# Guivernoir/ICS-WT-PhysicsEngine

Hardware: AMD Instinct MI355X
Metric: reactor-zone-steps/sec (higher is better)
Workload: dtype f64

## Files before the change

### ics-wt-physicsengine_amd/csrc/wt_device.hpp

```cpp
#pragma once
#include <hip/hip_runtime.h>
#include <stdint.h>
#include <type_traits>
#include "wt_sensors.hpp"
#include "wt_ctl.hpp"
#include "wt_inj.hpp"
#include "wt_alm.hpp"
#include "wt_det.hpp"
#include "wt_act.hpp"
#include "wt_dst.hpp"
#include "wt_scr.hpp"

namespace wt {

#ifdef WT_STAMPS
constexpr int WT_DIAG_SLOTS = 16;
#else
constexpr int WT_DIAG_SLOTS = 8;
#endif

constexpr int SPH = 0, SCL = 1, STT = 2;
#define WT_RARE(x) __builtin_expect(!!(x), 0)
#define WT_USUAL(x) __builtin_expect(!!(x), 1)
constexpr double RTOL = 1e-6, ATOL = 1e-8;
// ... 1220 lines not shown
            const double kd = k_diag(k, n.k_lo, khi_up);
            put(SPH, 2, row_pH(k, mix3(n.k_lo, khi_up, kd, n.H_lo, n.H_hi, b.H), b.H, b.iw));
            put(SCL, 2, row_Cl(k, mix3(n.k_lo, khi_up, kd, n.C_lo, n.C_hi, y[SCL]), y[SCL], kphi));
            put(STT, 2, row_T(k, mix3(n.k_lo, khi_up, kd, n.T_lo, Tx_hi, y[STT]), y[STT]));
        }
    }
}

template <bool ROW, int SP>
__device__ __forceinline__ void fd_col_reduce(const Lane &L, const FdCols &c, double &maxd, double &scale)
{
    maxd = -1.0; scale = 0.0;
#pragma unroll
    for (int q = 0; q < 3; ++q) {
        const bool dep_nb = (q == SP) || (SP == STT);
        const bool dep_own = dep_nb || (q == SCL && SP == SPH);
        if (!dep_own) continue;
        double d_lo = 0, s_lo = 0, d_hi = 0, s_hi = 0;
        if (dep_nb) {
            d_lo = from_lo<ROW, 1>(L, c.D[q][2]); s_lo = from_lo<ROW, 1>(L, c.S[q][2]);
            d_hi = from_hi<ROW, 1>(L, c.D[q][0]); s_hi = from_hi<ROW, 1>(L, c.S[q][0]);
        }
        if (dep_nb && L.has_lo && fabs(d_lo) > maxd) { maxd = fabs(d_lo); scale = s_lo; }
        if (fabs(c.D[q][1]) > maxd) { maxd = fabs(c.D[q][1]); scale = c.S[q][1]; }
        if (dep_nb && L.has_hi && fabs(d_hi) > maxd) { maxd = fabs(d_hi); scale = s_hi; }
    }
}

__device__ __forceinline__ double fd_step(double y, double fac, double ysc)
{
    return __dadd_rn(__dadd_rn(y, __dmul_rn(fac, ysc)), -y);
}

template <bool ROW, int SP, class KC>
__device__ __forceinline__ void num_jac_species(const Lane &L, const KC &kc, const RK &k, const double y[3], const double f[3],
                                                const ZoneProps &b, const FdBase &nb, double &fac, FdCols &cols, bool &bad, double &badval)
{
    const double fs = (f[SP] >= 0) ? 1.0 : -1.0;
    const double ysc = fs * fmax(ATOL, fabs(y[SP]));
    double h = fd_step(y[SP], fac, ysc);
    while (WT_RARE(h == 0)) { fac *= 10; h = fd_step(y[SP], fac, ysc); }
    fd_species_pass<ROW, SP>(L, kc, k, y, f, b, nb, h, true, true, cols, bad, badval);
    double maxd, scl;
    fd_col_reduce<ROW, SP>(L, cols, maxd, scl);
    const bool small = maxd < rc::NJ_REJECT * scl;
    if (WT_RARE(__ballot(small) != 0ull)) {
        const double nf = 10 * fac;
        const double hn = fd_step(y[SP], nf, ysc);
        FdCols c2;
        fd_species_pass<ROW, SP>(L, kc, k, y, f, b, nb, hn, small, false, c2, bad, badval);
        double md2, sc2;
        fd_col_reduce<ROW, SP>(L, c2, md2, sc2);
        const bool upd = small && (maxd * sc2 < md2 * scl);
        if (upd) { fac = nf; h = hn; maxd = md2; scl = sc2; }
        const int iu = upd ? 1 : 0;
        const int iu_lo = __shfl_up(iu, 1, 64), iu_hi = __shfl_down(iu, 1, 64);
        const bool upd_lo = L.has_lo && (iu_lo != 0), upd_hi = L.has_hi && (iu_hi != 0);
#pragma unroll
        for (int q = 0; q < 3; ++q) {
            if (upd_lo) cols.D[q][0] = c2.D[q][0];
            if (upd) cols.D[q][1] = c2.D[q][1];
            if (upd_hi) cols.D[q][2] = c2.D[q][2];
        }
    }
    const double h_lo = from_lo<ROW, 1>(L, h), h_hi = from_hi<ROW, 1>(L, h);
    const double ih0 = L.has_lo ? rcp(h_lo) : 0.0, ih1 = rcp(h), ih2 = L.has_hi ? rcp(h_hi) : 0.0;
#pragma unroll
    for (int q = 0; q < 3; ++q) { cols.D[q][0] *= ih0; cols.D[q][1] *= ih1; cols.D[q][2] *= ih2; }
    const bool sm = maxd < rc::NJ_SMALL * scl, bg = maxd > rc::NJ_BIG * scl;
    if (sm) fac *= 10;
    if (bg) fac *= 0.1;
    fac = fmax(fac, rc::NJ_MINF);
}

template <bool ROW, class KTP>
__device__ __forceinline__ void num_jac(const Lane &L, const RKStore &ks, KTP ktab, const double y[3], const double f[3],
                                        double fac[3], bool &have_fac, Jac &J, bool &bad, double &badval, bool &t_dense)
{
    if (!have_fac) { fac[0] = fac[1] = fac[2] = rc::NJ_F0; have_fac = true; }
    FdCols cols;
    ZoneProps b;
    FdBase nb;
    {
        const KT ct = load_kt(ktab());
        const PropT bpt = prop_T(ct, y[STT]);
        b.kT = bpt.kT; b.rho = bpt.rho;
    }
    {
        const KP cp = load_kp(ktab());
        const RK k = fetch_reactor(ks);
        const PropPH bpp = prop_pH(cp, k, y[SPH]);
        b.H = bpp.H; b.iw = bpp.iw; b.phi = bpp.phi; b.bpos = bpp.bpos;
        nb = fd_base<ROW>(L, k, y, b);
        num_jac_species<ROW, SPH>(L, cp, k, y, f, b, nb, fac[SPH], cols, bad, badval);
#pragma unroll
        for (int r = 0; r < 3; ++r) J.pp[r] = cols.D[SPH][r];
        J.cp = cols.D[SCL][1];
    }
    {
        const RK k = fetch_reactor(ks);
        num_jac_species<ROW, SCL>(L, 0, k, y, f, b, nb, fac[SCL], cols, bad, badval);
#pragma unroll
        for (int r = 0; r < 3; ++r) J.cc[r] = cols.D[SCL][r];
    }
    {
        const KT ct = load_kt(ktab());
        const RK k = fetch_reactor(ks);
        num_jac_species<ROW, STT>(L, ct, k, y, f, b, nb, fac[STT], cols, bad, badval);
#pragma unroll
        for (int r = 0; r < 3; ++r) { J.tt[r] = cols.D[STT][r]; J.pt[r] = cols.D[SPH][r]; J.ct[r] = cols.D[SCL][r]; }
        t_dense = jac_t_dense(J) || (ct.dense_bias != 0.0);
    }
}

template <bool ROW, int LV = 6>
__device__ __forceinline__ double rms3(const Lane &L, const double x[3], const double sc[3])
{
    double s = 0.0;
#pragma unroll
    for (int q = 0; q < 3; ++q) { const double v = x[q] * rcp(sc[q]); s += v * v; }
    return sqrt_k(div_by(seg_sum<ROW, LV>(L, s), L.d3n));
}

__device__ __forceinline__ double ulp_above(double t)
{
    return __longlong_as_double(__double_as_longlong(t) + 1) - t;
}

__device__ __forceinline__ double predict_factor(double h_abs, bool have_old, double h_abs_old,
                                                 double error_norm, double error_norm_old)
{
    double mult = 1.0;
    const double ie = rcp(error_norm);
    if (have_old && error_norm != 0) mult = h_abs * rcp(h_abs_old) * root4(error_norm_old * ie);
    return fmin(1.0, mult) * root4(ie);
}

struct Flag {
    uint32_t &w; const uint32_t m;
    __device__ __forceinline__ operator bool() const { return (w & m) != 0u; }
    __device__ __forceinline__ Flag &operator=(bool v) { w = v ? (w | m) : (w & ~m); return *this; }
    __device__ __forceinline__ Flag &operator=(const Flag &o) { return *this = (bool)o; }
    __device__ __forceinline__ Flag &operator|=(bool v) { w = v ? (w | m) : w; return *this; }
};

enum Phase : int {
    PH_OUTER_BEGIN = 0,
    PH_INIT_STEP,
    PH_F1,
    PH_STEP_BEGIN,
    PH_ATTEMPT,
    PH_NEWTON,
    PH_ERR_REFINE,
    PH_FNEW,
    PH_DONE
};

struct SolverCounters { int nfev, njev, nlu, nsteps, nrej; };

__device__ __forceinline__ void lane_geometry(int n, Lane &L)
{
    const int lane = threadIdx.x & 63;
    const int seg = lane / n;
    L.n = n; L.z = lane - seg * n;
    L.base = seg * n;
    L.a_me = lane << 3; L.xrow = nullptr;
    L.has_lo = L.z > 0; L.has_hi = L.z < n - 1;
#pragma unroll
    for (int l = 0; l < 7; ++l) {
        L.m_lo[l] = (L.z - (1 << l) >= 0) ? ~0u : 0u;
        L.m_hi[l] = (L.z + (1 << l) < n) ? ~0u : 0u;
        asm("" : "+v"(L.m_lo[l]));
        asm("" : "+v"(L.m_hi[l]));
    }
    L.segmask = ((n >= 64) ? ~0ull : ((1ull << n) - 1ull)) << L.base;
    {
        int top = 1;
        while (2 * top < n) top *= 2;
        const bool up = L.z >= top, has = up || (L.z + top < n);
        L.m_pt = has ? ~0u : 0u;
        asm("" : "+v"(L.m_pt));
    }
    L.d3n = {(double)(3 * n), 1.0 / (double)(3 * n)};
    L.d9n = {(double)(9 * n), 1.0 / (double)(9 * n)};
}

__device__ __forceinline__ bool lane_setup(int64_t r0, int64_t r1, int n, int R, Lane &L, int64_t &r)
{
    lane_geometry(n, L);
    const int seg = (threadIdx.x & 63) / n;
    r = r0 + (int64_t)blockIdx.x * R + seg;
    return (seg < R) && (r < r1);
}

template <int LV> struct LdsMap {
    static constexpr int RK_DOUBLES = RK_UNI * rk_maxr(LV) + rk_lane_doubles(LV);
    static constexpr int HIST_DOUBLES = rk_maxr(LV);
    static constexpr int F_DOUBLES = FSlots<LV>::LDS_SLOTS * 64;
    static constexpr int IO_DOUBLES = (int)((sizeof(wts::StepIO) + 7) / 8);
    static constexpr int TAIL_DOUBLES = F_DOUBLES > IO_DOUBLES ? F_DOUBLES : IO_DOUBLES;
    static constexpr int X_OFF = RK_DOUBLES + HIST_DOUBLES, X_DOUBLES = 64;
    static constexpr int F_OFF = (X_OFF + X_DOUBLES + 1) & ~1;
    static constexpr int TOTAL = F_OFF + TAIL_DOUBLES;
    static_assert(X_OFF >= (LV >= 2 ? (1 << (LV - 2)) : 0), "reads below the exchange row must stay inside the allocation");
};

typedef const __attribute__((address_space(4))) StepArgs *ArgPtr;
__device__ __forceinline__ ArgPtr fresh(ArgPtr p)
{
    asm volatile("" : "+s"(p));
    return p;
}

__device__ __forceinline__ int queue_resolve(ArgPtr a, int ticket)
{
    const int n_groups = a->n_groups;
    if (ticket < n_groups) return n_groups - 1 - ticket;
    const unsigned long long want = (unsigned long long)(unsigned)(ticket + 1);
    unsigned long long *slot = a->q_slots + (ticket - n_groups) % a->q_cap;
    for (int spin = 0; spin < (1 << 22); ++spin) {
        const unsigned long long w = __hip_atomic_load(slot, __ATOMIC_RELAXED, __HIP_MEMORY_SCOPE_AGENT);
        if ((w >> 32) == want) return (int)(w & 0xffffffffull);
        __builtin_amdgcn_s_sleep(2);
    }
    __hip_atomic_store(a->q_ctrl + Q_ERROR, 1, __ATOMIC_RELAXED, __HIP_MEMORY_SCOPE_AGENT);
    return -1;
}

__device__ __forceinline__ void queue_push(ArgPtr a, int group)
{
    int32_t *ctrl = a->q_ctrl;
    const int p = __hip_atomic_fetch_add(ctrl + Q_TAIL, 1, __ATOMIC_RELAXED, __HIP_MEMORY_SCOPE_AGENT);
    const unsigned long long w = ((unsigned long long)(unsigned)(a->n_groups + p + 1) << 32) | (unsigned)group;
    __hip_atomic_store(a->q_slots + p % a->q_cap, w, __ATOMIC_RELAXED, __HIP_MEMORY_SCOPE_AGENT);
    __hip_atomic_fetch_add(ctrl + Q_AVAIL, 1, __ATOMIC_RELEASE, __HIP_MEMORY_SCOPE_AGENT);
}

__device__ __forceinline__ int queue_next(ArgPtr pa, int own, bool hold, bool &exchanged)
{
    ArgPtr a = fresh(pa);
    const bool lane0 = (threadIdx.x & 63) == 0;
    int ticket = -1;
    if (lane0 && !(own >= 0 && hold)) {
        int32_t *avail = a->q_ctrl + Q_AVAIL;
        do {
            const int old = __hip_atomic_fetch_add(avail, -1, __ATOMIC_RELAXED, __HIP_MEMORY_SCOPE_AGENT);
            if (old > 0) { ticket = __hip_atomic_fetch_add(a->q_ctrl + Q_HEAD, 1, __ATOMIC_RELAXED, __HIP_MEMORY_SCOPE_AGENT); break; }
            __hip_atomic_fetch_add(avail, 1, __ATOMIC_RELAXED, __HIP_MEMORY_SCOPE_AGENT);
        } while (__hip_atomic_load(avail, __ATOMIC_RELAXED, __HIP_MEMORY_SCOPE_AGENT) > 0);
    }
    ticket = __builtin_amdgcn_readfirstlane(ticket);
    exchanged = ticket >= 0;
    if (ticket < 0) return own;
    if (own >= 0) {
        asm volatile("s_waitcnt vmcnt(0)" ::: "memory");
        __builtin_amdgcn_fence(__ATOMIC_RELEASE, "agent");
        asm volatile("s_waitcnt vmcnt(0)" ::: "memory");
    }
    int next = -1;
    if (lane0) {
        if (own >= 0) queue_push(a, own);
        next = queue_resolve(a, ticket);
    }
    return __builtin_amdgcn_readfirstlane(next);
}

template <bool ROW, int NS>
__device__ __forceinline__ void rhs_points(const Lane &L, const RKStore &ks, ArgPtr pa, const double (*y)[3], double (*F)[3], bool *bad)
{
    PropPH pp[NS]; PropT pt[NS];
    {
        ArgPtr a = fresh(pa);
        const KP c = load_kp(&a->kt);
        const RK k = fetch_reactor(ks);
        double x[NS];
#pragma unroll
        for (int s = 0; s < NS; ++s) x[s] = y[s][SPH];
        prop_pH_n<NS>(c, k, x, pp);
    }
    __builtin_amdgcn_sched_barrier(0);
    {
        ArgPtr a = fresh(pa);
        const KT c = load_kt(&a->kt);
        double x[NS];
#pragma unroll
        for (int s = 0; s < NS; ++s) x[s] = y[s][STT];
        prop_T_n<NS>(c, x, pt);
#pragma unroll
        for (int s = 0; s < NS; ++s) bad[s] = pt[s].bad;
    }
    {
        const RK k = fetch_reactor(ks);
#pragma unroll
        for (int s = 0; s < NS; ++s)
            rhs_rows<ROW>(L, k, pp[s].H, pp[s].iw, pp[s].bpos, pt[s].kT * pp[s].phi, pt[s].rho, y[s][SCL], y[s][STT], F[s]);
    }
}

template <int LV, bool ROW>
__device__ __forceinline__ void run_item(ArgPtr pa, const Lane &L, double *lds, int group, int step0, int cnt)
{
    using M = LdsMap<LV>;
    ArgPtr a = fresh(pa);
    const int n_zones = L.n, R = a->R;
    const int lane = threadIdx.x & 63, seg = lane / n_zones;
    const int64_t q_first = (int64_t)group * R;
    const int64_t q_end = a->q_ctrl ? a->N : a->r1;
    const bool present = (seg < R) && (q_first + seg < q_end);
    const int64_t r = present ? (int64_t)a->perm[q_first + seg] : 0;
    const int64_t idx = r * n_zones + L.z;
    const double dt = a->dt;
    const int step_limit = a->step_limit, sens_on = a->sens.on, plc_on = a->sens.plc_on;
    const bool want_diag = a->wave_diag != nullptr;
    const RKStore ks = {lds + seg, lds + RK_UNI * rk_maxr(LV) + lane, rk_maxr(LV), L.m_lo[0], L.m_hi[0], rk_lane_in_lds(LV)};
    int *hist0 = reinterpret_cast<int *>(lds + M::RK_DOUBLES);
    int *rix = hist0 + rk_maxr(LV);
    double *lds_factors = lds + M::F_OFF;
    wts::StepIO &io = *reinterpret_cast<wts::StepIO *>(lds_factors);

    double y0[3] = {7.0, 1.0, 20.0};
    double f[3] = {0, 0, 0};
    double t_out = 0;
    double dH = 0, dR = 0, dK = 0, badval = 0;
    double flow_used = 0;
    uint32_t st = 0;
    bool frozen = !present, f_valid = false, wrote_k = false, raised = false;
    int steps_done = 0, reads_done = 0, cost_acc = 0;
    SolverCounters last_cnt = {0, 0, 0, 0, 0};
    int diag_trips = 0, diag_newton = 0;
#ifdef WT_STAMPS
    int diag_fact = 0, diag_jac = 0, diag_f3 = 0;
#define WT_COUNT(c) ++(c)
#else
    constexpr int diag_fact = 0, diag_jac = 0, diag_f3 = 0;
#define WT_COUNT(c) do { } while (0)
#endif
#ifdef WT_STAMPS
    long long sec[8] = {0, 0, 0, 0, 0, 0, 0, 0}; long long tprev = __builtin_amdgcn_s_memtime();
#define WT_STAMP(i) do { const long long tn_ = __builtin_amdgcn_s_memtime(); sec[i] += tn_ - tprev; tprev = tn_; } while (0)
#else
#define WT_STAMP(i) do { } while (0)
#endif
    const long long clk0 = want_diag ? __builtin_amdgcn_s_memtime() : 0, wall0 = want_diag ? __builtin_amdgcn_s_memrealtime() : 0;
    if (present) {
        st = a->status[r];
        if (st & (ST_T_RANGE | ST_T_RANGE_POST)) frozen = true;
        y0[SPH] = a->pH[idx]; y0[SCL] = a->Cl[idx]; y0[STT] = a->T[idx];
        t_out = a->time[r];
        const double *bc = a->sched ? a->sched + (int64_t)(a->first_step + step0) * NB * a->N : a->bc;
        RK k0; load_reactor(a->par, bc, a->N, r, n_zones, k0); mask_reactor_for_lane(L, k0);
        park_reactor(ks, k0);
        if (sens_on && L.z == 0) hist0[seg] = a->sens.hist_value ? a->sens.hist_pos[r] : 0;
        if (L.z == 0) rix[seg] = (int)r;
    }

    for (int k = 0; k < cnt; ++k) {
        bool stepped = false;
        if (!frozen) {
          if (WT_RARE(seg_any(L, !(isfinite(y0[0]) && isfinite(y0[1]) && isfinite(y0[2]))))) { st |= ST_NONFINITE; frozen = true; }
          else {
            double yc[3], W[3][3];
            double aux[3] = {0, 0, 0};
            constexpr bool HELD = LV <= 5;
            typedef Held<HELD> AReg64;
            AReg64 Qa[3][3], y_old_a[3], sol_t_old_a, sol_h_a;
#pragma unroll
            for (int q = 0; q < 3; ++q) { y_old_a[q].init(); Qa[q][0].init(); Qa[q][1].init(); Qa[q][2].init(); }
            sol_t_old_a.init(); sol_h_a.init();
            Jac J;
            JacA<(LV <= 4)> ja; ja.init();
            FStore<LV> F;
            F.cell = (LdsDouble2 *)lds_factors + lane;
            uint32_t fl = 1u << 4;
            Flag have_fac{fl, 1u << 0}, have_old{fl, 1u << 1}, have_old_l{fl, 1u << 2}, have_sol{fl, 1u << 3}, current_jac{fl, 1u << 4},
                 have_lu{fl, 1u << 5}, rejected{fl, 1u << 6}, keep_h{fl, 1u << 7}, have_norm_old{fl, 1u << 8}, have_rate{fl, 1u << 9},
                 bad{fl, 1u << 10}, failed{fl, 1u << 11}, fv{fl, 1u << 12}, need_jac{fl, 1u << 13},
                 limit_hit{fl, 1u << 16}, pend_f{fl, 1u << 17}, jac_after_fnew{fl, 1u << 18},
                 j_dense{fl, 1u << 19};
            fv = f_valid;
            AReg64 fac_a[3]; fac_a[0].init(); fac_a[1].init(); fac_a[2].init();
            double t = t_out, t_bound = t_out + dt, max_step = fmin(dt, 10.0);
            double h = 0, t_new = 0, h_abs = 0, h_abs_l = 0, min_step = 0;
            AReg64 h_abs_old_a, err_old_a, h_abs_old_l_a, err_old_l_a;
            h_abs_old_a.init(); err_old_a.init(); h_abs_old_l_a.init(); err_old_l_a.init();
            int kk = 0, n_iter = 0; double dW_norm_old = 0, rate = 0;
            double error_norm = 0, safety = 0;
            double d0 = 0, d1 = 0, h0 = 0;
            SolverCounters cnt_s = {0, 0, 0, 0, 0};
            int attempts = 0;
            int badstage = 0;
            int phase = PH_OUTER_BEGIN;
#pragma unroll
            for (int q = 0; q < 3; ++q) { yc[q] = y0[q]; W[0][q] = W[1][q] = W[2][q] = 0.0; }

            auto initial_step_first_half = [&]() {
                double sc[3];
#pragma unroll
                for (int q = 0; q < 3; ++q) sc[q] = ATOL + fabs(yc[q]) * RTOL;
                d0 = rms3<ROW, LV>(L, yc, sc); d1 = rms3<ROW, LV>(L, f, sc);
                h0 = (d0 < 1e-5 || d1 < 1e-5) ? 1e-6 : 0.01 * d0 * rcp(d1);
                h0 = fmin(h0, fabs(t_bound - t));
#pragma unroll
                for (int q = 0; q < 3; ++q) aux[q] = yc[q] + h0 * f[q];
            };
            auto reject_step = [&]() {
                const double fct = predict_factor(h_abs_l, have_old_l, h_abs_old_l_a.get(), error_norm, err_old_l_a.get());
                h_abs_l *= fmax(MIN_FACTOR, safety * fct);
                have_lu = false; rejected = true; cnt_s.nrej++;
                phase = PH_ATTEMPT;
            };
            auto accept_step = [&]() {
                const bool recompute_jac = (n_iter > 2) && have_rate && (rate > 1e-3);
                double fct = predict_factor(h_abs_l, have_old_l, h_abs_old_l_a.get(), error_norm, err_old_l_a.get());
                fct = fmin(MAX_FACTOR, safety * fct);
                if (!recompute_jac && fct < 1.2) fct = 1.0; else have_lu = false;
                h_abs_old_a.set(h_abs);
                err_old_a.set(error_norm);
                have_old = true;
                h_abs = h_abs_l * fct;
                const KZ kz = lit_kz(); const KA ka = lit_ka();
#pragma unroll
                for (int q = 0; q < 3; ++q) {
                    const double z0 = kz.T00 * W[0][q] + kz.T01 * W[1][q] + kz.T02 * W[2][q];
                    const double z1 = kz.T10 * W[0][q] + kz.T11 * W[1][q] + kz.T12 * W[2][q];
                    const double z2 = W[0][q] + W[1][q];
                    y_old_a[q].set(yc[q]);
                    Qa[q][0].set(z0 * ka.P[0] + z1 * ka.P[3] + z2 * ka.P[6]);
                    Qa[q][1].set(z0 * ka.P[1] + z1 * ka.P[4] + z2 * ka.P[7]);
                    Qa[q][2].set(z0 * ka.P[2] + z1 * ka.P[5] + z2 * ka.P[8]);
                    yc[q] = yc[q] + z2;
                }
                sol_t_old_a.set(t); sol_h_a.set(t_new - t); have_sol = true;
                t = t_new;
                cnt_s.nsteps++; cnt_s.nfev++;
                pend_f = true; fv = false;
                current_jac = recompute_jac;
                const bool more = (t - t_bound) < 0;
                if (recompute_jac || !more) { jac_after_fnew = recompute_jac; phase = PH_FNEW; }
                else phase = PH_STEP_BEGIN;
            };

            if (fv) {
                cnt_s.nfev++;
                phase = PH_INIT_STEP;
            }

            WT_STAMP(0);
            while (true) {
                if (__ballot(phase != PH_DONE) == 0ull) break;
                if (phase == PH_INIT_STEP) {
                    initial_step_first_half();
                    phase = PH_F1;
                }
                if (phase == PH_STEP_BEGIN) {
                    min_step = 10 * fabs(ulp_above(t));
                    if (h_abs > max_step) { h_abs_l = max_step; have_old_l = false; }
                    else if (h_abs < min_step) { h_abs_l = min_step; have_old_l = false; }
                    else { h_abs_l = h_abs; have_old_l = have_old; h_abs_old_l_a.set(h_abs_old_a.get()); err_old_l_a.set(err_old_a.get()); }
                    rejected = false; keep_h = false;
                    phase = PH_ATTEMPT;
                }
                if (phase == PH_ATTEMPT) {
                    if (!keep_h) {
                        if (WT_RARE(step_limit > 0 && attempts >= step_limit)) { failed = true; limit_hit = true; phase = PH_DONE; }
                        else if (WT_RARE(h_abs_l < min_step)) { failed = true; phase = PH_DONE; }
                        else {
                            attempts++;
                            h = h_abs_l;
                            t_new = t + h;
                            if (t_new - t_bound > 0) t_new = t_bound;
                            h = t_new - t;
                            h_abs_l = fabs(h);
                        }
                    }
                    if (phase == PH_ATTEMPT) {
                        keep_h = false;
                        double Z0[3][3];
                        if (!have_sol) {
#pragma unroll
                            for (int s = 0; s < 3; ++s)
#pragma unroll
                                for (int q = 0; q < 3; ++q) Z0[s][q] = 0.0;
                        } else {
                            const double sol_t_old = sol_t_old_a.get(), isol = rcp(sol_h_a.get());
                            double Q[3][3], y_old[3];
#pragma unroll
                            for (int q = 0; q < 3; ++q) { y_old[q] = y_old_a[q].get(); Q[q][0] = Qa[q][0].get(); Q[q][1] = Qa[q][1].get(); Q[q][2] = Qa[q][2].get(); }
                            const KG kg = load_kg(&fresh(pa)->rt);
                            const double cs[3] = {kg.C0, kg.C1, 1.0};
#pragma unroll
                            for (int s = 0; s < 3; ++s) {
                                const double x = ((t + h * cs[s]) - sol_t_old) * isol;
                                const double p1 = x * x, p2 = p1 * x;
#pragma unroll
                                for (int q = 0; q < 3; ++q)
                                    Z0[s][q] = (__builtin_fma(Q[q][2], p2, __builtin_fma(Q[q][0], x, Q[q][1] * p1)) + y_old[q]) - yc[q];
                            }
                        }
                        const KN kn0 = load_kn(&fresh(pa)->rt);
#pragma unroll
                        for (int q = 0; q < 3; ++q) {
                            W[0][q] = kn0.TI[0] * Z0[0][q] + kn0.TI[1] * Z0[1][q] + kn0.TI[2] * Z0[2][q];
                            W[1][q] = kn0.TI[3] * Z0[0][q] + kn0.TI[4] * Z0[1][q] + kn0.TI[5] * Z0[2][q];
                            W[2][q] = kn0.TI[6] * Z0[0][q] + kn0.TI[7] * Z0[1][q] + kn0.TI[8] * Z0[2][q];
                        }
                        kk = 0; have_norm_old = false; have_rate = false; rate = 0.0;
                        phase = PH_NEWTON;
                    }
                }
                WT_STAMP(1);
#ifdef WT_STAMPS
                if (__ballot(phase == PH_NEWTON && !have_lu) != 0ull) WT_COUNT(diag_fact);
#endif
                if (phase == PH_NEWTON && !have_lu) {
                    { Jac Jb; ja.bands(Jb); factorize<ROW, LV>(L, Jb, h, F); } have_lu = true; cnt_s.nlu += 2;
                }

                WT_STAMP(2);
                const bool newton = (phase == PH_NEWTON);
                diag_trips++; if (__ballot(newton) != 0ull) diag_newton++;
                const bool eval0 = (phase == PH_OUTER_BEGIN || phase == PH_F1 || phase == PH_ERR_REFINE || phase == PH_FNEW || newton);
                const bool eval3 = newton && pend_f;
                double ye[3][3], Fe[3][3];
#pragma unroll
                for (int q = 0; q < 3; ++q) {
                    double p0 = yc[q];
                    if (phase == PH_F1) p0 = aux[q];
                    if (phase == PH_ERR_REFINE) p0 = yc[q] + aux[q];
                    ye[0][q] = p0;
                }
                auto stage_points = [&]() {
                    const KZ kzp = load_kz(&fresh(pa)->rt);
#pragma unroll
                    for (int q = 0; q < 3; ++q) {
                        const double z0 = kzp.T00 * W[0][q] + kzp.T01 * W[1][q] + kzp.T02 * W[2][q];
                        const double z1 = kzp.T10 * W[0][q] + kzp.T11 * W[1][q] + kzp.T12 * W[2][q];
                        const double z2 = W[0][q] + W[1][q];
                        if (newton) ye[0][q] = yc[q] + z0;
                        ye[1][q] = yc[q] + z1; ye[2][q] = yc[q] + z2;
                    }
                };
                if constexpr (LV >= 5) stage_points();
                bool b0 = false, b1 = false, b2 = false, b3 = false;
                if (__ballot(newton) != 0ull) {
                    if constexpr (LV < 5) stage_points();
                    bool bb[3];
                    rhs_points<ROW, 3>(L, ks, pa, ye, Fe, bb);
                    b0 = bb[0] && eval0; b1 = bb[1] && newton; b2 = bb[2] && newton;
                    if (eval0 && phase != PH_FNEW) cnt_s.nfev++;
                    if (newton) cnt_s.nfev += 2;
                } else if (__ballot(eval0) != 0ull) {
                    bool bb[1];
                    rhs_points<ROW, 1>(L, ks, pa, ye, Fe, bb);
                    b0 = bb[0] && eval0;
                    if (eval0 && phase != PH_FNEW) cnt_s.nfev++;
                }
                if (__ballot(eval3) != 0ull) {
                    WT_COUNT(diag_f3);
                    double fy[1][3]; bool bb[1];
                    rhs_points<ROW, 1>(L, ks, pa, &yc, fy, bb);
                    b3 = bb[0] && eval3;
                    if (eval3) {
                        pend_f = false;
#pragma unroll
                        for (int q = 0; q < 3; ++q) f[q] = fy[0][q];
                    }
                }
                if (WT_RARE(__ballot(b0 || b1 || b2 || b3) != 0ull)) {
                    const bool mine = b0 || b1 || b2 || b3;
                    if (mine && !bad) {
                        badstage = b3 ? 0 : (b0 ? 1 : (b1 ? 2 : 3));
                        badval = b3 ? yc[STT] : (b0 ? ye[0][STT] : (b1 ? ye[1][STT] : ye[2][STT]));
                    }
                    bad |= mine;
                    if (seg_any(L, bad)) { raised = true; phase = PH_DONE; }
                }

                WT_STAMP(3);
                if (WT_RARE(phase == PH_OUTER_BEGIN)) {
#pragma unroll
                    for (int q = 0; q < 3; ++q) f[q] = Fe[0][q];
                    phase = PH_INIT_STEP;
                } else if (phase == PH_F1) {
                    double sc[3], df[3];
#pragma unroll
                    for (int q = 0; q < 3; ++q) { sc[q] = ATOL + fabs(yc[q]) * RTOL; df[q] = Fe[0][q] - f[q]; }
                    const double d2 = rms3<ROW, LV>(L, df, sc) * rcp(h0);
                    double h1;
                    if (d1 <= 1e-15 && d2 <= 1e-15) h1 = fmax(1e-6, h0 * 1e-3);
                    else h1 = root4(0.01 * rcp(fmax(d1, d2)));
                    h_abs = fmin(fmin(100 * h0, h1), fmin(fabs(t_bound - t), max_step));
                    need_jac = true;
                    phase = PH_STEP_BEGIN;
                } else if (phase == PH_NEWTON) {
                    Jac Jc; ja.coupling(Jc);
                    bool finite = true;
#pragma unroll
                    for (int s = 0; s < 3; ++s)
#pragma unroll
                        for (int q = 0; q < 3; ++q) finite = finite && isfinite(Fe[s][q]);
                    bool conv = false, diverged = false;
                    if (WT_RARE(!seg_all(L, finite))) {
                        diverged = true;
                    } else {
                        const double ih = rcp(h);
                        const RTabPtr rt = &fresh(pa)->rt;
                        const KN kn = load_kn(rt); const KZ kz = load_kz(rt);
                        const double M_real = kn.mu_r * ih, Mcr = kn.mu_cr * ih, Mci = kn.mu_ci * ih;
                        double fr[3], fcr[3], fci[3], scale[3];
#pragma unroll
                        for (int q = 0; q < 3; ++q) {
                            scale[q] = kz.atol + fabs(yc[q]) * kz.rtol;
                            fr[q] = (Fe[0][q] * kn.TI[0] + Fe[1][q] * kn.TI[1] + Fe[2][q] * kn.TI[2]) - M_real * W[0][q];
                            const double re = Fe[0][q] * kn.TI[3] + Fe[1][q] * kn.TI[4] + Fe[2][q] * kn.TI[5];
                            const double im = Fe[0][q] * kn.TI[6] + Fe[1][q] * kn.TI[7] + Fe[2][q] * kn.TI[8];
                            fcr[q] = re - (Mcr * W[1][q] - Mci * W[2][q]);
                            fci[q] = im - (Mcr * W[2][q] + Mci * W[1][q]);
                        }
                        solve_rc<ROW, LV>(L, Jc, F, fr, fcr, fci, __ballot(j_dense) == 0ull);
                        double ssum = 0.0;
#pragma unroll
                        for (int q = 0; q < 3; ++q) {
                            const double is = rcp(scale[q]);
                            const double u = fr[q] * is, v = fcr[q] * is, w = fci[q] * is;
                            ssum += u * u + v * v + w * w;
                        }
                        const double dW_norm = sqrt_k(div_by(seg_sum<ROW, LV>(L, ssum), L.d9n));
                        if (have_norm_old) { rate = dW_norm * rcp(dW_norm_old); have_rate = true; }
                        const double i1r = rcp(1 - rate);
                        if (have_rate && (rate >= 1 || powi6(rate, NEWTON_MAXITER - kk) * i1r * dW_norm > kn.newton_tol)) {
                            diverged = true;
                        } else {
#pragma unroll
                            for (int q = 0; q < 3; ++q) { W[0][q] += fr[q]; W[1][q] += fcr[q]; W[2][q] += fci[q]; }
                            if (dW_norm == 0 || (have_rate && rate * i1r * dW_norm < kn.newton_tol)) conv = true;
                            dW_norm_old = dW_norm; have_norm_old = true;
                        }
                    }
                    n_iter = kk + 1;
                    kk++;
                    if (!conv && !diverged && kk == NEWTON_MAXITER) diverged = true;
                    if (WT_RARE(diverged)) {
                        if (current_jac) { h_abs_l *= 0.5; have_lu = false; cnt_s.nrej++; phase = PH_ATTEMPT; }
                        else { need_jac = true; current_jac = true; have_lu = false; keep_h = true; phase = PH_ATTEMPT; }
                    } else if (conv) {
                        double err[3], esc[3];
                        const double ih_e = rcp(h);
                        const KZ kze = lit_kz(); const KE ke = lit_ke();
#pragma unroll
                        for (int q = 0; q < 3; ++q) {
                            const double z0 = kze.T00 * W[0][q] + kze.T01 * W[1][q] + kze.T02 * W[2][q];
                            const double z1 = kze.T10 * W[0][q] + kze.T11 * W[1][q] + kze.T12 * W[2][q];
                            const double z2 = W[0][q] + W[1][q];
                            const double ZE = (z0 * ke.E0 + z1 * ke.E1 + z2 * ke.E2) * ih_e;
                            err[q] = f[q] + ZE;
                            esc[q] = kze.atol + fmax(fabs(yc[q]), fabs(yc[q] + z2)) * kze.rtol;
                        }
                        solve_real<ROW, LV>(L, Jc, F, err, __ballot(j_dense) == 0ull);
                        error_norm = rms3<ROW, LV>(L, err, esc);
                        safety = 0.9 * (2 * NEWTON_MAXITER + 1) / (2 * NEWTON_MAXITER + n_iter);
                        if (WT_RARE(rejected && error_norm > 1)) {
#pragma unroll
                            for (int q = 0; q < 3; ++q) aux[q] = err[q];
                            phase = PH_ERR_REFINE;
                        } else if (WT_RARE(error_norm > 1)) {
                            reject_step();
                        } else {
                            accept_step();
                        }
                    }
                } else if (WT_RARE(phase == PH_ERR_REFINE)) {
                    Jac Jc; ja.coupling(Jc);
                    double err[3], esc[3];
                    const double ih_e = rcp(h);
                    const KZ kze = lit_kz(); const KE ke = lit_ke();
#pragma unroll
                    for (int q = 0; q < 3; ++q) {
                        const double z0 = kze.T00 * W[0][q] + kze.T01 * W[1][q] + kze.T02 * W[2][q];
                        const double z1 = kze.T10 * W[0][q] + kze.T11 * W[1][q] + kze.T12 * W[2][q];
                        const double z2 = W[0][q] + W[1][q];
                        const double ZE = (z0 * ke.E0 + z1 * ke.E1 + z2 * ke.E2) * ih_e;
                        err[q] = Fe[0][q] + ZE;
                        esc[q] = kze.atol + fmax(fabs(yc[q]), fabs(yc[q] + z2)) * kze.rtol;
                    }
                    solve_real<ROW, LV>(L, Jc, F, err, __ballot(j_dense) == 0ull);
                    error_norm = rms3<ROW, LV>(L, err, esc);
                    if (error_norm > 1) reject_step(); else accept_step();
                } else if (phase == PH_FNEW) {
#pragma unroll
                    for (int q = 0; q < 3; ++q) f[q] = Fe[0][q];
                    pend_f = false;
                    fv = true;
                    if (jac_after_fnew) { need_jac = true; jac_after_fnew = false; }
                    phase = ((t - t_bound) < 0) ? PH_STEP_BEGIN : PH_DONE;
                }

                WT_STAMP(4);
#ifdef WT_STAMPS
                if (__ballot(need_jac) != 0ull) WT_COUNT(diag_jac);
#endif
                if (need_jac) {
                    bool jbad = false, hf = have_fac, jd = false; double jval = 0;
                    asm volatile("" ::: "memory");
                    double fac[3] = {fac_a[0].get(), fac_a[1].get(), fac_a[2].get()};
                    num_jac<ROW>(L, ks, [&]() { return &fresh(pa)->kt; }, yc, f, fac, hf, J, jbad, jval, jd); cnt_s.njev++;
                    fac_a[0].set(fac[0]); fac_a[1].set(fac[1]); fac_a[2].set(fac[2]);
                    have_fac = hf;
                    j_dense = jd;
                    ja.put(J);
                    need_jac = false;
                    if (WT_RARE(seg_any(L, jbad))) {
                        if (jbad && !bad) { badstage = 4; badval = jval; }
                        bad |= jbad; raised = true; phase = PH_DONE;
                    }
                }
                WT_STAMP(5);
            }
            last_cnt = cnt_s;
            cost_acc += cnt_s.nfev;

            if (WT_RARE(raised)) {
                st |= ST_T_RANGE; frozen = true;
                double v = badval; int best = 1 << 30;
#pragma unroll 1
                for (int sidx = 0; sidx < 5; ++sidx) {
                    const unsigned long long m = __ballot(bad && badstage == sidx) & L.segmask;
                    if (m != 0ull && best == (1 << 30)) { best = sidx; v = __shfl(badval, (int)__builtin_ctzll(m), 64); }
                }
                badval = v;
                raised = false;
            } else {
                if (failed) st |= ST_SOLVER_FAILED;
                if (limit_hit) st |= ST_STEP_LIMIT;
#pragma unroll
                for (int q = 0; q < 3; ++q) y0[q] = yc[q];
                stepped = true; steps_done++;
                t_out = t_out + dt;
                flow_used = ks.uni[15 * ks.stride];
                double dHv; PropT pt;
                {
                    ArgPtr a2 = fresh(pa);
                    const KP cp = load_kp(&a2->kt); const KT ct = load_kt(&a2->kt);
                    dHv = exp10_k(cp, -y0[SPH]); pt = prop_T(ct, y0[STT]);
                }
                dH = dHv;
                dR = pt.rho;
                bool clamped = false;
                if (WT_RARE(seg_any(L, pt.bad))) {
                    st |= ST_T_RANGE_POST; frozen = true;
                    const unsigned long long m = __ballot(pt.bad) & L.segmask;
                    badval = __shfl(y0[STT], (int)__builtin_ctzll(m), 64);
                } else {
                    dK = pt.kT; wrote_k = true;
                    if (WT_RARE(seg_any(L, y0[SPH] < 0 || y0[SPH] > 14))) { st |= ST_CLAMP_PH; y0[SPH] = fmin(fmax(y0[SPH], 0.0), 14.0); clamped = true; }
                    if (WT_RARE(seg_any(L, y0[SCL] < 0))) { st |= ST_CLAMP_CL; y0[SCL] = fmax(y0[SCL], 0.0); clamped = true; }
                    if (WT_RARE(seg_any(L, y0[STT] < 0 || y0[STT] > 100))) { st |= ST_CLAMP_T; y0[STT] = fmin(fmax(y0[STT], 0.0), 100.0); clamped = true; }
                    f_valid = fv && !clamped && !failed;
                }
            }
          }
        }

        WT_STAMP(6);
        if constexpr (prog_in_item(LV)) {
          if (WT_RARE(fresh(pa)->scr.on)) {
            ArgPtr s = fresh(pa);
            static_assert(M::TAIL_DOUBLES >= wtsc::STAGE_DOUBLES, "the score program stages the zones' state in the factor store");
            const bool live = present && stepped && !(st & ST_T_RANGE_POST);
            wtsc::evaluate(s->scr, live, L.z, n_zones, lane, L.base, r, t_out, y0, lds_factors,
                           s->scr.step0 + s->first_step + step0 + k);
          }
        }
        if constexpr (prog_in_item(LV)) {
          if (WT_RARE(fresh(pa)->dst.on)) {
            ArgPtr d = fresh(pa);
            const bool live = present && stepped && !(st & ST_T_RANGE_POST);
            if (live && L.z == 0) wtd::evaluate(d->dst, r, t_out, d->bc, d->N, ExpK());
            __syncthreads();
            if (live) {
                RK k1; load_reactor(d->par, d->bc, d->N, r, n_zones, k1); mask_reactor_for_lane(L, k1);
                park_reactor(ks, k1);
                f_valid = false;
            }
          }
        }
        if (sens_on) {
            ArgPtr b = fresh(pa);
            __syncthreads();
            if (seg < R) {
                const bool live = stepped && !(st & ST_T_RANGE_POST);
                if (L.z == 0) {
                    io.stepped[seg] = live ? 1 : 0;
                    if (live) reads_done++;
                    io.t_after[seg] = t_out;
                    io.tap[0][seg] = (float)y0[SPH]; io.tap[2][seg] = (float)y0[SCL]; io.tap[4][seg] = (float)y0[STT];
                    io.tap[6][seg] = (float)flow_used;
                }
                if (!L.has_hi) { io.tap[1][seg] = (float)y0[SPH]; io.tap[3][seg] = (float)y0[SCL]; io.tap[5][seg] = (float)y0[STT]; }
            }
            __syncthreads();
            wts::suite_step(b->sens, io, rix, R, hist0, k);
            if (plc_on) {
                const int gs = b->first_step + step0 + k;
                const bool scan = ((gs + 1) % b->sens.scan_every == 0) || (gs + 1 == b->call_steps);
                __syncthreads();
                if (lane < R && io.stepped[lane]) {
                    const int64_t rr = rix[lane];
                    const double lt = b->sens.pack.loop_time[rr];
                    if (scan) {
                        const bool inj = prog_in_item(LV) && WT_RARE(fresh(pa)->inj.on);
                        if (inj) wti::tamper_sensors(fresh(pa)->inj, rr, &io.val[0][lane], &io.fault[0][lane], wts::RMAX, lt + dt);
                        wtp::pack_inputs(b->sens.pack, rr, &io.val[0][lane], &io.fault[0][lane], wts::RMAX, lt);
                        double c[3];
                        const bool act = prog_in_item(LV) && WT_RARE(fresh(pa)->act.on);
                        const double row0 = act ? b->sens.cmd.bc[rr] : 0.0;
                        double inlet_v;
                        if (inj) inlet_v = wtp::apply_commands(b->sens.cmd, rr, c, wti::command_tamper(fresh(pa)->inj, rr, lt + dt));
                        else inlet_v = wtp::apply_commands(b->sens.cmd, rr, c);
                        if (prog_in_item(LV) && WT_RARE(fresh(pa)->alm.on)) wta::override_commands(fresh(pa)->alm, b->sens.cmd, rr, c);
                        if (act) wtv::actuate(fresh(pa)->act, b->sens.cmd, rr, c, inlet_v, row0, lt + dt);
                        io.cmd[0][lane] = c[0]; io.cmd[1][lane] = c[1]; io.cmd[2][lane] = c[2];
                    }
                    b->sens.pack.loop_time[rr] = lt + dt;
                }
                if (scan && WT_RARE(fresh(pa)->ctl.on) && lane < R && io.stepped[lane]) {
                    ArgPtr cp = fresh(pa);
                    const int64_t rr = rix[lane];
                    wtc::pi_execute(cp->ctl, rr, &io.val[0][lane], &io.fault[0][lane], wts::RMAX, cp->sens.pack.loop_time[rr]);
                }
                if (prog_in_item(LV) && scan && WT_RARE(fresh(pa)->alm.on) && lane < R && io.stepped[lane]) {
                    ArgPtr ap = fresh(pa);
                    const int64_t rr = rix[lane];
                    wta::evaluate(ap->alm, rr, ap->sens.N, &io.val[0][lane], &io.fault[0][lane], wts::RMAX, ap->sens.out_value,
                                  ap->sens.out_fault, ap->sens.pack.loop_time[rr]);
                }
                if constexpr (prog_in_item(LV)) {
                  if (scan && WT_RARE(fresh(pa)->det.on) && lane < R && io.stepped[lane]) {
                    ArgPtr dp = fresh(pa);
                    const int64_t rr = rix[lane];
                    wtk::evaluate(dp->det, rr, dp->sens.N, &io.val[0][lane], &io.fault[0][lane], wts::RMAX, dp->sens.out_value,
                                  dp->sens.out_fault, dp->sens.pack.loop_time[rr]);
                  }
                }
                if (scan) {
                    __syncthreads();
                    if (present && io.stepped[seg]) {
                        RK k0; load_reactor(b->par, b->bc, b->N, r, n_zones, k0, &io.cmd[0][seg], wts::RMAX); mask_reactor_for_lane(L, k0);
                        park_reactor(ks, k0);
                        f_valid = false;
                    }
// ... 293 lines not shown
```

Before: 1.622 billion.

## Evaluate post-accept RHS inline after step instead of separate FNEW phase

Removes the PH_FNEW phase and the deferred pend_f evaluation fused into the next Newton iteration. After an accepted step, f(y) is now evaluated in the same loop trip via a dedicated rhs call guarded by f_due, followed immediately by a Jacobian request if recompute was set. This saves a loop trip per step when the Jacobian is recomputed or at the step boundary. The trade-off is that every accepted step now pays a separate single-point RHS call instead of overlapping it with the Newton stage evaluation, and wave divergence may change.

```diff
diff --git a/ics-wt-physicsengine_amd/csrc/wt_device.hpp b/ics-wt-physicsengine_amd/csrc/wt_device.hpp
--- a/ics-wt-physicsengine_amd/csrc/wt_device.hpp
+++ b/ics-wt-physicsengine_amd/csrc/wt_device.hpp
@@ -1396,7 +1396,6 @@
     PH_ATTEMPT,
     PH_NEWTON,
     PH_ERR_REFINE,
-    PH_FNEW,
     PH_DONE
 };
 
@@ -1619,7 +1618,7 @@
             Flag have_fac{fl, 1u << 0}, have_old{fl, 1u << 1}, have_old_l{fl, 1u << 2}, have_sol{fl, 1u << 3}, current_jac{fl, 1u << 4},
                  have_lu{fl, 1u << 5}, rejected{fl, 1u << 6}, keep_h{fl, 1u << 7}, have_norm_old{fl, 1u << 8}, have_rate{fl, 1u << 9},
                  bad{fl, 1u << 10}, failed{fl, 1u << 11}, fv{fl, 1u << 12}, need_jac{fl, 1u << 13},
-                 limit_hit{fl, 1u << 16}, pend_f{fl, 1u << 17}, jac_after_fnew{fl, 1u << 18},
+                 limit_hit{fl, 1u << 16}, f_due{fl, 1u << 17},
                  j_dense{fl, 1u << 19};
             fv = f_valid;
             AReg64 fac_a[3]; fac_a[0].init(); fac_a[1].init(); fac_a[2].init();
@@ -1677,11 +1676,9 @@
                 sol_t_old_a.set(t); sol_h_a.set(t_new - t); have_sol = true;
                 t = t_new;
                 cnt_s.nsteps++; cnt_s.nfev++;
-                pend_f = true; fv = false;
+                f_due = true; fv = false;
                 current_jac = recompute_jac;
-                const bool more = (t - t_bound) < 0;
-                if (recompute_jac || !more) { jac_after_fnew = recompute_jac; phase = PH_FNEW; }
-                else phase = PH_STEP_BEGIN;
+                phase = ((t - t_bound) < 0) ? PH_STEP_BEGIN : PH_DONE;
             };
 
             if (fv) {
@@ -1763,8 +1760,7 @@
                 WT_STAMP(2);
                 const bool newton = (phase == PH_NEWTON);
                 diag_trips++; if (__ballot(newton) != 0ull) diag_newton++;
-                const bool eval0 = (phase == PH_OUTER_BEGIN || phase == PH_F1 || phase == PH_ERR_REFINE || phase == PH_FNEW || newton);
-                const bool eval3 = newton && pend_f;
+                const bool eval0 = (phase == PH_OUTER_BEGIN || phase == PH_F1 || phase == PH_ERR_REFINE || newton);
                 double ye[3][3], Fe[3][3];
 #pragma unroll
                 for (int q = 0; q < 3; ++q) {
@@ -1785,36 +1781,25 @@
                     }
                 };
                 if constexpr (LV >= 5) stage_points();
-                bool b0 = false, b1 = false, b2 = false, b3 = false;
+                bool b0 = false, b1 = false, b2 = false;
                 if (__ballot(newton) != 0ull) {
                     if constexpr (LV < 5) stage_points();
                     bool bb[3];
                     rhs_points<ROW, 3>(L, ks, pa, ye, Fe, bb);
                     b0 = bb[0] && eval0; b1 = bb[1] && newton; b2 = bb[2] && newton;
-                    if (eval0 && phase != PH_FNEW) cnt_s.nfev++;
+                    if (eval0) cnt_s.nfev++;
                     if (newton) cnt_s.nfev += 2;
                 } else if (__ballot(eval0) != 0ull) {
                     bool bb[1];
                     rhs_points<ROW, 1>(L, ks, pa, ye, Fe, bb);
                     b0 = bb[0] && eval0;
-                    if (eval0 && phase != PH_FNEW) cnt_s.nfev++;
+                    if (eval0) cnt_s.nfev++;
                 }
-                if (__ballot(eval3) != 0ull) {
-                    WT_COUNT(diag_f3);
-                    double fy[1][3]; bool bb[1];
-                    rhs_points<ROW, 1>(L, ks, pa, &yc, fy, bb);
-                    b3 = bb[0] && eval3;
-                    if (eval3) {
-                        pend_f = false;
-#pragma unroll
-                        for (int q = 0; q < 3; ++q) f[q] = fy[0][q];
-                    }
-                }
-                if (WT_RARE(__ballot(b0 || b1 || b2 || b3) != 0ull)) {
-                    const bool mine = b0 || b1 || b2 || b3;
+                if (WT_RARE(__ballot(b0 || b1 || b2) != 0ull)) {
+                    const bool mine = b0 || b1 || b2;
                     if (mine && !bad) {
-                        badstage = b3 ? 0 : (b0 ? 1 : (b1 ? 2 : 3));
-                        badval = b3 ? yc[STT] : (b0 ? ye[0][STT] : (b1 ? ye[1][STT] : ye[2][STT]));
+                        badstage = b0 ? 1 : (b1 ? 2 : 3);
+                        badval = b0 ? ye[0][STT] : (b1 ? ye[1][STT] : ye[2][STT]);
                     }
                     bad |= mine;
                     if (seg_any(L, bad)) { raised = true; phase = PH_DONE; }
@@ -1930,16 +1915,27 @@
                     solve_real<ROW, LV>(L, Jc, F, err, __ballot(j_dense) == 0ull);
                     error_norm = rms3<ROW, LV>(L, err, esc);
                     if (error_norm > 1) reject_step(); else accept_step();
-                } else if (phase == PH_FNEW) {
-#pragma unroll
-                    for (int q = 0; q < 3; ++q) f[q] = Fe[0][q];
-                    pend_f = false;
-                    fv = true;
-                    if (jac_after_fnew) { need_jac = true; jac_after_fnew = false; }
-                    phase = ((t - t_bound) < 0) ? PH_STEP_BEGIN : PH_DONE;
                 }
 
                 WT_STAMP(4);
+                if (__ballot(f_due) != 0ull) {
+                    WT_COUNT(diag_f3);
+                    double fy[1][3]; bool bb[1];
+                    rhs_points<ROW, 1>(L, ks, pa, &yc, fy, bb);
+                    const bool b3 = bb[0] && f_due;
+                    if (WT_RARE(__ballot(b3) != 0ull)) {
+                        if (b3 && !bad) { badstage = 0; badval = yc[STT]; }
+                        bad |= b3;
+                        if (seg_any(L, bad)) { raised = true; phase = PH_DONE; }
+                    }
+                    if (f_due && !raised) {
+#pragma unroll
+                        for (int q = 0; q < 3; ++q) f[q] = fy[0][q];
+                        fv = true;
+                        if (current_jac) need_jac = true;
+                    }
+                    f_due = false;
+                }
 #ifdef WT_STAMPS
                 if (__ballot(need_jac) != 0ull) WT_COUNT(diag_jac);
 #endif
```

After: 1.637 billion, median of 3. About the same (+0.9%).
